# OmerMersin/video-stab

Measured on AMD Instinct MI355X. Metric: stabilized frames/sec @1080p (whole job; warp-stage HBM GB/s in roofline), higher is better.
Workload: dtype u8

## Files before the change

### video-stab_amd/csrc/k_lk.hip

```cpp
#include "vs_common.h"

namespace vsd {
namespace {

constexpr int MAX_LEVELS = 8;

struct LKArgs {
    LKLevel levels[MAX_LEVELS];
    int max_level;
    const float* prev_pts;
    float* next_pts;
    uint8_t* status;
    float* err;
    int n;
    const int32_t* d_n;
    int win;
    int max_count;
    double eps2;
};

template <int CTRL>
__device__ __forceinline__ int dpp_mov(int v) {
    return __builtin_amdgcn_update_dpp(0, v, CTRL, 0xF, 0xF, true);
}
__device__ __forceinline__ int wave_sum_i32(int v) {
    v += dpp_mov<0xB1>(v);
    v += dpp_mov<0x4E>(v);
    v += dpp_mov<0x141>(v);
    v += dpp_mov<0x140>(v);
    return __builtin_amdgcn_readlane(v, 0) + __builtin_amdgcn_readlane(v, 16) +
           __builtin_amdgcn_readlane(v, 32) + __builtin_amdgcn_readlane(v, 48);
}
template <int CTRL>
__device__ __forceinline__ long long dpp_mov64(long long v) {
    const int lo = dpp_mov<CTRL>((int)(unsigned)(unsigned long long)v);
    const int hi = dpp_mov<CTRL>((int)((unsigned long long)v >> 32));
    return (long long)(((unsigned long long)(unsigned)hi << 32) | (unsigned)lo);
}
__device__ __forceinline__ long long wave_sum(int p) {
    long long v = p;
    v += dpp_mov64<0xB1>(v);
    v += dpp_mov64<0x4E>(v);
    v += dpp_mov64<0x141>(v);
    v += dpp_mov64<0x140>(v);
    const int lo = (int)(unsigned)(unsigned long long)v, hi = (int)((unsigned long long)v >> 32);
    long long t = 0;
#pragma unroll
    for (int r = 0; r < 64; r += 16) {
        const unsigned l = (unsigned)__builtin_amdgcn_readlane(lo, r);
        const unsigned h = (unsigned)__builtin_amdgcn_readlane(hi, r);
        t += (long long)(((unsigned long long)h << 32) | l);
    }
    return t;
}

__device__ __forceinline__ int descale(int x, int n) { return (x + (1 << (n - 1))) >> n; }

struct Weights { int w00, w01, w10, w11; };

__device__ __forceinline__ Weights make_weights(float a, float b) {
    Weights w;
    w.w00 = f_round((1.f - a) * (1.f - b) * 16384.f);
    w.w01 = f_round(a * (1.f - b) * 16384.f);
    w.w10 = f_round((1.f - a) * b * 16384.f);
    w.w11 = 16384 - w.w00 - w.w01 - w.w10;
    return w;
}

typedef const __attribute__((address_space(1))) uint8_t* gmem_u8;
__device__ __forceinline__ gmem_u8 uniform_global(const uint8_t* p) {
    const unsigned long long v = (unsigned long long)p;
    const unsigned lo = (unsigned)__builtin_amdgcn_readfirstlane((int)(unsigned)v), hi = (unsigned)__builtin_amdgcn_readfirstlane((int)(unsigned)(v >> 32));
    return (gmem_u8)(((unsigned long long)hi << 32) | lo);
}

constexpr int LK_MARGIN = 6;
constexpr int LK_WIN_MAX = 31;



__device__ __forceinline__ void divmod_small(int i, int d, float inv_d, int& q, int& r) {
    q = (int)(((float)i + 0.5f) * inv_d);
    r = i - q * d;
}

template <int NPX>
__device__ __forceinline__ void lk_track(const LKArgs& a, const int pt) {
    constexpr int WM = NPX <= 4 ? 16 : (NPX <= 7 ? 21 : LK_WIN_MAX);
    constexpr int PWM = WM + 1, RWM = WM + 1 + 2 * LK_MARGIN;
    constexpr int DR = NPX <= 7 ? 3 : 5;
    constexpr int PPM = (PWM + 2 + 3) & ~3;
    constexpr int SRM = (PWM + 1 + 3) / 4, NGM = (PWM + DR - 1) / DR;
    static_assert(SRM * NGM <= 64, "one derivative round per level");
    constexpr int PN = (PPM * (PWM + 2) + 63) / 64, RN = (RWM * RWM + 63) / 64;
    constexpr int PBYTES = (PN * 64 > PPM * (NGM * DR + 2) + 4 ? PN * 64 : PPM * (NGM * DR + 2) + 4);
    __shared__ __attribute__((aligned(16))) uint8_t pI_[4 + PBYTES];
    uint8_t* const pI = pI_ + 4;
    __shared__ __attribute__((aligned(16))) short2 pD[(PWM + 1) * PPM];
    __shared__ uint8_t region[RN * 64];
    const int lane = threadIdx.x;
    int n = a.n;
    if (a.d_n) { int dn = *a.d_n; n = dn < n ? dn : n; }
    if (pt >= n) return;
    const int win = a.win, area = win * win;
    const int PW = win + 1, PP = (PW + 2 + 3) & ~3;
    const int RW = win + 1 + 2 * LK_MARGIN;
    const float inv_pp = 1.0f / (float)PP, inv_rw = 1.0f / (float)RW, inv_win = 1.0f / (float)win;
    uint32_t off[NPX];
#pragma unroll
    for (int k = 0; k < NPX; k++) {
        const int p = lane + 64 * k;
        int yy = 0, xx = 0;
        if (p < area) divmod_small(p, win, inv_win, yy, xx);
        off[k] = (uint32_t)((yy + 1) * PP + xx + 1) | ((uint32_t)(yy * RW + xx) << 16);
    }
#define LK_VALID(k) (lane + 64 * (k) < area)
#define LK_POFF(k) ((int)(off[k] & 0xFFFFu))
#define LK_ROFF(k) ((int)(off[k] >> 16))
    int p_y0, p_x0, p_sy, p_sx, r_y0, r_x0, r_sy, r_sx;
    divmod_small(lane, PP, inv_pp, p_y0, p_x0);
    divmod_small(64, PP, inv_pp, p_sy, p_sx);
    divmod_small(lane, RW, inv_rw, r_y0, r_x0);
    divmod_small(64, RW, inv_rw, r_sy, r_sx);
    const float halfWin = (win - 1) * 0.5f;
    const float FLT_SCALE = 1.f / (1 << 20);
    const float px0 = a.prev_pts[2 * pt], py0 = a.prev_pts[2 * pt + 1];
    float outx = 0.f, outy = 0.f;
    int status = 1;
    float err = 0.f;

    for (int level = a.max_level; level >= 0; level--) {
        const LKLevel L = a.levels[level];
        const float scale = (float)(1. / (double)(1 << level));
        float prevx = px0 * scale, prevy = py0 * scale;
        if (level == a.max_level) { outx = prevx; outy = prevy; }
        else { outx = outx * 2.f; outy = outy * 2.f; }
        prevx -= halfWin; prevy -= halfWin;
        const int ipx = f_floor(prevx), ipy = f_floor(prevy);
        if (ipx < -win || ipx >= L.w || ipy < -win || ipy >= L.h) {
            if (level == 0) { status = 0; err = 0.f; }
            continue;
        }
        float cx = outx - halfWin, cy = outy - halfWin;
        int rx0 = f_floor(cx) - LK_MARGIN, ry0 = f_floor(cy) - LK_MARGIN;
        __syncthreads();
        const int pcount = PP * (PW + 2);
        if (ipx >= 1 && ipy >= 1 && ipx - 1 + PP <= L.w && ipy + PW + 1 <= L.h) {
            const gmem_u8 pbase = uniform_global(L.prev + ((size_t)(ipy - 1) * L.stride + (ipx - 1)));
            constexpr int PB_ = 10;
            int y = p_y0, x = p_x0;
#pragma unroll
            for (int k0 = 0; k0 < PN; k0 += PB_) {
                uint8_t vI[PB_];
#pragma unroll
                for (int k = k0; k < k0 + PB_ && k < PN; k++) {
                    const bool ok = lane + 64 * k < pcount;
                    vI[k - k0] = pbase[ok ? (uint32_t)(y * (int)L.stride + x) : 0u];
                    x += p_sx; y += p_sy;
                    if (x >= PP) { x -= PP; y++; }
                }
#pragma unroll
                for (int k = k0; k < k0 + PB_ && k < PN; k++) pI[lane + 64 * k] = vI[k - k0];
                __builtin_amdgcn_sched_barrier(0);
            }
        } else {
            int y = p_y0, x = p_x0;
            for (int i = lane; i < pcount; i += 64) {
                const int X = ipx - 1 + x, Y = ipy - 1 + y;
                pI[i] = L.prev[(size_t)reflect101(Y, L.h) * L.stride + reflect101(X, L.w)];
                x += p_sx; y += p_sy;
                if (x >= PP) { x -= PP; y++; }
            }
        }
        auto stage_region = [&]() {
            const bool inside = rx0 >= 0 && ry0 >= 0 && rx0 + RW <= L.w && ry0 + RW <= L.h;
            int y = r_y0, x = r_x0;
            asm volatile("" : "+v"(x), "+v"(y));
            if (inside) {
                const gmem_u8 rbase = uniform_global(L.next + ((size_t)ry0 * L.stride + rx0));
                constexpr int RB_ = 10;
#pragma unroll
                for (int k0 = 0; k0 < RN; k0 += RB_) {
                    uint8_t vR[RB_];
#pragma unroll
                    for (int k = k0; k < k0 + RB_ && k < RN; k++) {
                        const bool ok = lane + 64 * k < RW * RW;
                        vR[k - k0] = rbase[ok ? (uint32_t)(y * (int)L.stride + x) : 0u];
                        x += r_sx; y += r_sy;
                        if (x >= RW) { x -= RW; y++; }
                    }
#pragma unroll
                    for (int k = k0; k < k0 + RB_ && k < RN; k++) region[lane + 64 * k] = vR[k - k0];
                    __builtin_amdgcn_sched_barrier(0);
                }
            } else {
                for (int i = lane; i < RW * RW; i += 64) {
                    const int X = rx0 + x, Y = ry0 + y;
                    region[i] = L.next[(size_t)reflect101(Y, L.h) * L.stride + reflect101(X, L.w)];
                    x += r_sx; y += r_sy;
                    if (x >= RW) { x -= RW; y++; }
                }
            }
        };
        stage_region();
        __syncthreads();
        {
            const int sr = (PW + 1 + 3) >> 2;
            int g, c;
            divmod_small(lane, sr, 1.0f / (float)sr, g, c);
            const int y = 1 + g * DR, x = 4 * c;
            if (y <= PW) {
                const bool masked = !(ipx >= 0 && ipy >= 0 && ipx + PW <= L.w && ipy + PW <= L.h);
                int t[3][6];
                auto load_row = [&](int j, int* tj) {
                    const uint32_t* q = reinterpret_cast<const uint32_t*>(pI + j * PP) + c;
                    const uint32_t lo = q[-1], mid = q[0], hi = q[1];
                    tj[0] = lo >> 24;
                    tj[1] = mid & 255u; tj[2] = (mid >> 8) & 255u; tj[3] = (mid >> 16) & 255u; tj[4] = mid >> 24;
                    tj[5] = hi & 255u;
                };
                load_row(y - 1, t[0]);
                load_row(y, t[1]);
#pragma unroll
                for (int r = 0; r < DR; r++) {
                    const int* t0 = t[r % 3];
                    const int* t1 = t[(r + 1) % 3];
                    int* t2 = t[(r + 2) % 3];
                    load_row(y + r + 1, t2);
                    int av[6], bv[6];
#pragma unroll
                    for (int k = 0; k < 6; k++) {
                        av[k] = (t0[k] + t2[k]) * 3 + t1[k] * 10;
                        bv[k] = t2[k] - t0[k];
                    }
                    uint32_t o[4];
#pragma unroll
                    for (int k = 0; k < 4; k++) {
                        const int dx = av[k + 2] - av[k], dy = (bv[k + 2] + bv[k]) * 3 + bv[k + 1] * 10;
                        o[k] = ((uint32_t)dx & 0xFFFFu) | ((uint32_t)dy << 16);
                        if (masked && ((unsigned)(ipx - 1 + x + k) >= (unsigned)L.w || (unsigned)(ipy - 1 + y + r) >= (unsigned)L.h)) o[k] = 0u;
                    }
                    if (y + r <= PW) *reinterpret_cast<uint4*>(&pD[(y + r) * PP + x]) = make_uint4(o[0], o[1], o[2], o[3]);
                    __builtin_amdgcn_sched_barrier(0);
                }
            }
        }
        __syncthreads();
#pragma unroll
        for (int k = 0; k < NPX; k++) asm volatile("" : "+v"(off[k]));
        Weights wt = make_weights(prevx - ipx, prevy - ipy);
        short Iw[NPX], Ix[NPX], Iy[NPX];
        int pA11 = 0, pA12 = 0, pA22 = 0;
#pragma unroll
        for (int k = 0; k < NPX; k++) {
            const int o = LK_POFF(k);
            int ival = descale(__mul24((int)pI[o], wt.w00) + __mul24((int)pI[o + 1], wt.w01) +
                               __mul24((int)pI[o + PP], wt.w10) + __mul24((int)pI[o + PP + 1], wt.w11), 9);
            const short2 d00 = pD[o], d01 = pD[o + 1], d10 = pD[o + PP], d11 = pD[o + PP + 1];
            int ixval = descale(__mul24((int)d00.x, wt.w00) + __mul24((int)d01.x, wt.w01) +
                                __mul24((int)d10.x, wt.w10) + __mul24((int)d11.x, wt.w11), 14);
            int iyval = descale(__mul24((int)d00.y, wt.w00) + __mul24((int)d01.y, wt.w01) +
                                __mul24((int)d10.y, wt.w10) + __mul24((int)d11.y, wt.w11), 14);
            if (!LK_VALID(k)) { ival = 0; ixval = 0; iyval = 0; }
            Iw[k] = (short)ival; Ix[k] = (short)ixval; Iy[k] = (short)iyval;
            pA11 += __mul24(ixval, ixval);
            pA12 += __mul24(ixval, iyval);
            pA22 += __mul24(iyval, iyval);
        }
        const long long sA11 = wave_sum(pA11), sA12 = wave_sum(pA12), sA22 = wave_sum(pA22);
        const float A11 = (float)sA11 * FLT_SCALE, A12 = (float)sA12 * FLT_SCALE, A22 = (float)sA22 * FLT_SCALE;
        float D = A11 * A22 - A12 * A12;
        const float minEig = (A22 + A11 - sqrtf((A11 - A22) * (A11 - A22) + 4.f * A12 * A12)) /
                             (float)(2 * win * win);
        if (minEig < 1e-4f || D < FLT_EPSILON) {
            if (level == 0) status = 0;
            continue;
        }
        D = 1.f / D;
        float pdx = 0.f, pdy = 0.f;
        for (int j = 0; j < a.max_count; j++) {
            const int inx = f_floor(cx), iny = f_floor(cy);
            if (inx < -win || inx >= L.w || iny < -win || iny >= L.h) {
                if (level == 0) status = 0;
                break;
            }
            wt = make_weights(cx - inx, cy - iny);
            int lx = inx - rx0, ly = iny - ry0;
            if (!(lx >= 0 && ly >= 0 && lx + win + 1 <= RW && ly + win + 1 <= RW)) {
                __syncthreads();
                rx0 = inx - LK_MARGIN; ry0 = iny - LK_MARGIN;
                stage_region();
                __syncthreads();
                lx = LK_MARGIN; ly = LK_MARGIN;
            }
            int pb1 = 0, pb2 = 0;
            {
                const int rbase = ly * RW + lx;
#pragma unroll
                for (int k = 0; k < NPX; k++) {
                    const uint8_t* r0 = &region[rbase + LK_ROFF(k)];
                    const int v = descale(__mul24((int)r0[0], wt.w00) + __mul24((int)r0[1], wt.w01) +
                                          __mul24((int)r0[RW], wt.w10) + __mul24((int)r0[RW + 1], wt.w11), 9);
                    const int diff = v - Iw[k];
                    pb1 += __mul24(diff, (int)Ix[k]);
                    pb2 += __mul24(diff, (int)Iy[k]);
                }
            }
            const long long sb1 = wave_sum(pb1), sb2 = wave_sum(pb2);
            const float b1 = (float)sb1 * FLT_SCALE, b2 = (float)sb2 * FLT_SCALE;
            const float dx = (A12 * b2 - A22 * b1) * D;
            const float dy = (A12 * b1 - A11 * b2) * D;
            cx += dx; cy += dy;
            outx = cx + halfWin; outy = cy + halfWin;
            if ((double)dx * (double)dx + (double)dy * (double)dy <= a.eps2) break;
            if (j > 0 && (double)fabsf(dx + pdx) < 0.01 && (double)fabsf(dy + pdy) < 0.01) {
                outx -= dx * 0.5f; outy -= dy * 0.5f;
                break;
            }
            pdx = dx; pdy = dy;
        }
        if (status && level == 0) {
            const float npx = outx - halfWin, npy = outy - halfWin;
            const int inx = f_floor(npx), iny = f_floor(npy);
            if (inx < -win || inx >= L.w || iny < -win || iny >= L.h) {
                status = 0;
            } else {
                wt = make_weights(npx - inx, npy - iny);
                int lx = inx - rx0, ly = iny - ry0;
                if (!(lx >= 0 && ly >= 0 && lx + win + 1 <= RW && ly + win + 1 <= RW)) {
                    __syncthreads();
                    rx0 = inx - LK_MARGIN; ry0 = iny - LK_MARGIN;
                    stage_region();
                    __syncthreads();
                    lx = LK_MARGIN; ly = LK_MARGIN;
                }
                int es = 0;
                {
                    const int rbase = ly * RW + lx;
#pragma unroll
                    for (int k = 0; k < NPX; k++) {
                        const uint8_t* r0 = &region[rbase + LK_ROFF(k)];
                        const int v = descale(__mul24((int)r0[0], wt.w00) + __mul24((int)r0[1], wt.w01) +
                                              __mul24((int)r0[RW], wt.w10) + __mul24((int)r0[RW + 1], wt.w11), 9);
                        const int diff = v - Iw[k];
                        es += LK_VALID(k) ? (diff < 0 ? -diff : diff) : 0;
                    }
                }
                const long long est = wave_sum(es);
                err = (float)est * 1.f / (float)(32 * win * win);
            }
        }
    }
#undef LK_VALID
#undef LK_POFF
#undef LK_ROFF
    if (lane == 0) {
        a.next_pts[2 * pt] = outx;
        a.next_pts[2 * pt + 1] = outy;
        a.status[pt] = (uint8_t)status;
        a.err[pt] = err;
    }
}

template <int NPX>
__global__ __launch_bounds__(64) void lk_kernel(LKArgs a) { lk_track<NPX>(a, blockIdx.x); }

template <int NPX>
__global__ __launch_bounds__(64) void lk_batch_kernel(const LKArgs* __restrict__ table) {
    lk_track<NPX>(table[blockIdx.y], blockIdx.x);
}

int fill_lk_args(LKArgs& a, const LKLevel* levels, int max_level, const float* d_prev_pts, int n, const int32_t* d_n,
                 float* d_next_pts, uint8_t* d_status, float* d_err, int win, int max_iters, double eps) {
    if (!levels || max_level < 0 || max_level >= MAX_LEVELS || n < 0 || win < 3 || win > 31 ||
        !d_prev_pts || !d_next_pts || !d_status || !d_err) {
        set_last_error("pyr_lk: invalid argument (3 <= win <= 31, max_level < 8)");
        return VS_ERR_INVALID_ARG;
    }
    for (int i = 0; i <= max_level; i++) a.levels[i] = levels[i];
    for (int i = max_level + 1; i < MAX_LEVELS; i++) a.levels[i] = levels[max_level];
    a.max_level = max_level;
    a.prev_pts = d_prev_pts; a.next_pts = d_next_pts; a.status = d_status; a.err = d_err;
    a.n = n; a.d_n = d_n; a.win = win;
    a.max_count = max_iters < 0 ? 0 : (max_iters > 100 ? 100 : max_iters);
    double e = eps < 0 ? 0. : (eps > 10. ? 10. : eps);
    a.eps2 = e * e;
    return VS_OK;
}

}

size_t lk_item_bytes() { return sizeof(LKArgs); }

int lk_fill_item(void* host_item, const LKLevel* levels, int max_level, const float* d_prev_pts, int n,
                 const int32_t* d_n, float* d_next_pts, uint8_t* d_status, float* d_err, int win, int max_iters,
                 double eps) {
    return fill_lk_args(*static_cast<LKArgs*>(host_item), levels, max_level, d_prev_pts, n, d_n, d_next_pts, d_status,
                        d_err, win, max_iters, eps);
}

int launch_pyr_lk_batch(const void* d_table, int items, int n_max, int win, hipStream_t st) {
    if (!d_table || items < 1 || items > 65535 || n_max < 0 || win < 3 || win > 31) {
        set_last_error("pyr_lk_batch: invalid argument");
        return VS_ERR_INVALID_ARG;
    }
    if (n_max == 0) return VS_OK;
    const LKArgs* t = static_cast<const LKArgs*>(d_table);
    const int npx = (win * win + 63) / 64;
    dim3 grid(n_max, items), block(64);
    if (npx <= 4) hipLaunchKernelGGL(lk_batch_kernel<4>, grid, block, 0, st, t);
    else if (npx <= 7) hipLaunchKernelGGL(lk_batch_kernel<7>, grid, block, 0, st, t);
    else hipLaunchKernelGGL(lk_batch_kernel<16>, grid, block, 0, st, t);
    VS_HIP_TRY(hipGetLastError());
    return VS_OK;
}

int launch_pyr_lk(const LKLevel* levels, int max_level, const float* d_prev_pts, int n,
                  const int32_t* d_n, float* d_next_pts, uint8_t* d_status, float* d_err, int win,
                  int max_iters, double eps, hipStream_t st) {
    LKArgs a;
    VS_TRY(fill_lk_args(a, levels, max_level, d_prev_pts, n, d_n, d_next_pts, d_status, d_err, win, max_iters, eps));
    if (n == 0) return VS_OK;
    const int npx = (win * win + 63) / 64;
    dim3 grid(n), block(64);
    if (npx <= 4) hipLaunchKernelGGL(lk_kernel<4>, grid, block, 0, st, a);
    else if (npx <= 7) hipLaunchKernelGGL(lk_kernel<7>, grid, block, 0, st, a);
    else hipLaunchKernelGGL(lk_kernel<16>, grid, block, 0, st, a);
    VS_HIP_TRY(hipGetLastError());
    return VS_OK;
}

int run_pyr_lk_op(const uint8_t* d_prev, const uint8_t* d_next, size_t stride, int w, int h,
                  const float* d_prev_pts, int n, float* d_next_pts, uint8_t* d_status,
                  float* d_err, int win, int max_level, int max_iters, double eps, hipStream_t st) {
    if (!d_prev || !d_next || w <= 0 || h <= 0 || max_level < 0 || max_level >= MAX_LEVELS) {
        set_last_error("pyr_lk: invalid argument");
        return VS_ERR_INVALID_ARG;
    }
    int lw[MAX_LEVELS], lh[MAX_LEVELS];
    int levels = 0;
    {
        int sw = w, sh = h;
        for (int level = 0; level <= max_level; level++) {
            lw[level] = sw; lh[level] = sh;
            levels = level;
            sw = (sw + 1) / 2; sh = (sh + 1) / 2;
            if (sw <= win || sh <= win) break;
        }
    }
    size_t img_bytes = 0;
    for (int i = 1; i <= levels; i++) img_bytes += (size_t)lw[i] * lh[i];
    uint8_t* scratch = nullptr;
    VS_HIP_TRY(hipMalloc((void**)&scratch, 2 * img_bytes + 64));
    LKLevel L[MAX_LEVELS];
    uint8_t* pp = scratch;
    uint8_t* pn = scratch + img_bytes;
    int rc = VS_OK;
    for (int i = 0; i <= levels && rc == VS_OK; i++) {
        L[i].w = lw[i]; L[i].h = lh[i];
        if (i == 0) { L[i].prev = d_prev; L[i].next = d_next; L[i].stride = stride; }
        else {
            rc = launch_pyr_down(L[i - 1].prev, L[i - 1].stride, lw[i - 1], lh[i - 1], pp, lw[i], st);
            if (rc == VS_OK) rc = launch_pyr_down(L[i - 1].next, L[i - 1].stride, lw[i - 1], lh[i - 1], pn, lw[i], st);
            L[i].prev = pp; L[i].next = pn; L[i].stride = lw[i];
            pp += (size_t)lw[i] * lh[i]; pn += (size_t)lw[i] * lh[i];
        }
    }
    if (rc == VS_OK) rc = launch_pyr_lk(L, levels, d_prev_pts, n, nullptr, d_next_pts, d_status, d_err, win, max_iters, eps, st);
    hipError_t e = hipStreamSynchronize(st);
    (void)hipFree(scratch);
    if (rc == VS_OK && e != hipSuccess) { set_last_error(hipGetErrorString(e)); rc = VS_ERR_HIP; }
    return rc;
}

}
```

Baseline: 126,300.

## Stage LK patches with 32-bit loads and shorten 64-bit wave reductions

Patch and search-region staging in the pyramidal LK tracker now uses unaligned 32-bit global loads into a row-padded (multiple-of-4) shared layout instead of per-byte loads. This cuts the number of memory instructions per staging pass, and region indexing is updated to the new pitch. The wave reduction now runs its first butterfly steps in 32-bit and only switches to 64-bit when the window size could overflow. This cuts DPP and readlane work per reduction. The padded region reads a few extra columns, which changes the inside-bounds check, and the fallback path now recomputes divmod per element.

```diff
diff --git a/video-stab_amd/csrc/k_lk.hip b/video-stab_amd/csrc/k_lk.hip
--- a/video-stab_amd/csrc/k_lk.hip
+++ b/video-stab_amd/csrc/k_lk.hip
@@ -23,25 +23,33 @@
 __device__ __forceinline__ int dpp_mov(int v) {
     return __builtin_amdgcn_update_dpp(0, v, CTRL, 0xF, 0xF, true);
 }
-__device__ __forceinline__ int wave_sum_i32(int v) {
-    v += dpp_mov<0xB1>(v);
-    v += dpp_mov<0x4E>(v);
-    v += dpp_mov<0x141>(v);
-    v += dpp_mov<0x140>(v);
-    return __builtin_amdgcn_readlane(v, 0) + __builtin_amdgcn_readlane(v, 16) +
-           __builtin_amdgcn_readlane(v, 32) + __builtin_amdgcn_readlane(v, 48);
-}
 template <int CTRL>
 __device__ __forceinline__ long long dpp_mov64(long long v) {
     const int lo = dpp_mov<CTRL>((int)(unsigned)(unsigned long long)v);
     const int hi = dpp_mov<CTRL>((int)((unsigned long long)v >> 32));
     return (long long)(((unsigned long long)(unsigned)hi << 32) | (unsigned)lo);
 }
+constexpr long long LK_LANE_TERM_MAX = 8160ll * 4081ll;
+template <int NPX> struct WaveSumSteps {
+    static constexpr int S = NPX <= 4 ? 4 : (NPX <= 7 ? 3 : 2);
+    static_assert(NPX <= 16 && (long long)NPX * LK_LANE_TERM_MAX * (1 << S) <= 2147483647ll, "the 32-bit butterfly steps must not overflow");
+};
+template <int S>
 __device__ __forceinline__ long long wave_sum(int p) {
-    long long v = p;
-    v += dpp_mov64<0xB1>(v);
-    v += dpp_mov64<0x4E>(v);
-    v += dpp_mov64<0x141>(v);
+    static_assert(S >= 2 && S <= 4, "");
+    unsigned u = (unsigned)p;
+    u += (unsigned)dpp_mov<0xB1>((int)u);
+    u += (unsigned)dpp_mov<0x4E>((int)u);
+    if (S >= 3) u += (unsigned)dpp_mov<0x141>((int)u);
+    if (S >= 4) u += (unsigned)dpp_mov<0x140>((int)u);
+    if (S >= 4) {
+        long long t = 0;
+#pragma unroll
+        for (int r = 0; r < 64; r += 16) t += (long long)__builtin_amdgcn_readlane((int)u, r);
+        return t;
+    }
+    long long v = (int)u;
+    if (S < 3) v += dpp_mov64<0x141>(v);
     v += dpp_mov64<0x140>(v);
     const int lo = (int)(unsigned)(unsigned long long)v, hi = (int)((unsigned long long)v >> 32);
     long long t = 0;
@@ -73,6 +81,9 @@
     const unsigned lo = (unsigned)__builtin_amdgcn_readfirstlane((int)(unsigned)v), hi = (unsigned)__builtin_amdgcn_readfirstlane((int)(unsigned)(v >> 32));
     return (gmem_u8)(((unsigned long long)hi << 32) | lo);
 }
+
+typedef uint32_t __attribute__((aligned(1))) u32_unaligned;
+typedef const __attribute__((address_space(1))) u32_unaligned* gmem_u32u;
 
 constexpr int LK_MARGIN = 6;
 constexpr int LK_WIN_MAX = 31;
@@ -92,12 +103,15 @@
     constexpr int PPM = (PWM + 2 + 3) & ~3;
     constexpr int SRM = (PWM + 1 + 3) / 4, NGM = (PWM + DR - 1) / DR;
     static_assert(SRM * NGM <= 64, "one derivative round per level");
-    constexpr int PN = (PPM * (PWM + 2) + 63) / 64, RN = (RWM * RWM + 63) / 64;
-    constexpr int PBYTES = (PN * 64 > PPM * (NGM * DR + 2) + 4 ? PN * 64 : PPM * (NGM * DR + 2) + 4);
+    constexpr int RDM = (RWM + 3) / 4;
+    constexpr int PN = ((PPM / 4) * (PWM + 2) + 63) / 64, RN = (RDM * RWM + 63) / 64;
+    constexpr int PBYTES = (PN * 256 > PPM * (NGM * DR + 2) + 4 ? PN * 256 : PPM * (NGM * DR + 2) + 4);
+    static_assert((WM - 1) * 4 * RDM + (WM - 1) < 65536 && (WM + 1) * PPM < 65536, "packed window offsets are 16 bits each");
+    constexpr int WS = WaveSumSteps<NPX>::S;
     __shared__ __attribute__((aligned(16))) uint8_t pI_[4 + PBYTES];
     uint8_t* const pI = pI_ + 4;
     __shared__ __attribute__((aligned(16))) short2 pD[(PWM + 1) * PPM];
-    __shared__ uint8_t region[RN * 64];
+    __shared__ __attribute__((aligned(16))) uint8_t region[RN * 256];
     const int lane = threadIdx.x;
     int n = a.n;
     if (a.d_n) { int dn = *a.d_n; n = dn < n ? dn : n; }
@@ -105,6 +119,7 @@
     const int win = a.win, area = win * win;
     const int PW = win + 1, PP = (PW + 2 + 3) & ~3;
     const int RW = win + 1 + 2 * LK_MARGIN;
+    const int PD = PP >> 2, RD = (RW + 3) >> 2, RP = 4 * RD;
     const float inv_pp = 1.0f / (float)PP, inv_rw = 1.0f / (float)RW, inv_win = 1.0f / (float)win;
     uint32_t off[NPX];
 #pragma unroll
@@ -112,16 +127,16 @@
         const int p = lane + 64 * k;
         int yy = 0, xx = 0;
         if (p < area) divmod_small(p, win, inv_win, yy, xx);
-        off[k] = (uint32_t)((yy + 1) * PP + xx + 1) | ((uint32_t)(yy * RW + xx) << 16);
+        off[k] = (uint32_t)((yy + 1) * PP + xx + 1) | ((uint32_t)(yy * RP + xx) << 16);
     }
 #define LK_VALID(k) (lane + 64 * (k) < area)
 #define LK_POFF(k) ((int)(off[k] & 0xFFFFu))
 #define LK_ROFF(k) ((int)(off[k] >> 16))
     int p_y0, p_x0, p_sy, p_sx, r_y0, r_x0, r_sy, r_sx;
-    divmod_small(lane, PP, inv_pp, p_y0, p_x0);
-    divmod_small(64, PP, inv_pp, p_sy, p_sx);
-    divmod_small(lane, RW, inv_rw, r_y0, r_x0);
-    divmod_small(64, RW, inv_rw, r_sy, r_sx);
+    divmod_small(lane, PD, 1.0f / (float)PD, p_y0, p_x0);
+    divmod_small(64, PD, 1.0f / (float)PD, p_sy, p_sx);
+    divmod_small(lane, RD, 1.0f / (float)RD, r_y0, r_x0);
+    divmod_small(64, RD, 1.0f / (float)RD, r_sy, r_sx);
     const float halfWin = (win - 1) * 0.5f;
     const float FLT_SCALE = 1.f / (1 << 20);
     const float px0 = a.prev_pts[2 * pt], py0 = a.prev_pts[2 * pt + 1];
@@ -147,58 +162,48 @@
         const int pcount = PP * (PW + 2);
         if (ipx >= 1 && ipy >= 1 && ipx - 1 + PP <= L.w && ipy + PW + 1 <= L.h) {
             const gmem_u8 pbase = uniform_global(L.prev + ((size_t)(ipy - 1) * L.stride + (ipx - 1)));
-            constexpr int PB_ = 10;
+            uint32_t vI[PN];
             int y = p_y0, x = p_x0;
 #pragma unroll
-            for (int k0 = 0; k0 < PN; k0 += PB_) {
-                uint8_t vI[PB_];
-#pragma unroll
-                for (int k = k0; k < k0 + PB_ && k < PN; k++) {
-                    const bool ok = lane + 64 * k < pcount;
-                    vI[k - k0] = pbase[ok ? (uint32_t)(y * (int)L.stride + x) : 0u];
-                    x += p_sx; y += p_sy;
-                    if (x >= PP) { x -= PP; y++; }
-                }
-#pragma unroll
-                for (int k = k0; k < k0 + PB_ && k < PN; k++) pI[lane + 64 * k] = vI[k - k0];
-                __builtin_amdgcn_sched_barrier(0);
-            }
+            for (int k = 0; k < PN; k++) {
+                const bool ok = lane + 64 * k < (pcount >> 2);
+                vI[k] = *(gmem_u32u)(pbase + (ok ? (uint32_t)(y * (int)L.stride + 4 * x) : 0u));
+                x += p_sx; y += p_sy;
+                if (x >= PD) { x -= PD; y++; }
+            }
+#pragma unroll
+            for (int k = 0; k < PN; k++) reinterpret_cast<uint32_t*>(pI)[lane + 64 * k] = vI[k];
+            __builtin_amdgcn_sched_barrier(0);
         } else {
-            int y = p_y0, x = p_x0;
             for (int i = lane; i < pcount; i += 64) {
+                int y, x;
+                divmod_small(i, PP, inv_pp, y, x);
                 const int X = ipx - 1 + x, Y = ipy - 1 + y;
                 pI[i] = L.prev[(size_t)reflect101(Y, L.h) * L.stride + reflect101(X, L.w)];
-                x += p_sx; y += p_sy;
-                if (x >= PP) { x -= PP; y++; }
             }
         }
         auto stage_region = [&]() {
-            const bool inside = rx0 >= 0 && ry0 >= 0 && rx0 + RW <= L.w && ry0 + RW <= L.h;
+            const bool inside = rx0 >= 0 && ry0 >= 0 && rx0 + RP <= L.w && ry0 + RW <= L.h;
             int y = r_y0, x = r_x0;
             asm volatile("" : "+v"(x), "+v"(y));
             if (inside) {
                 const gmem_u8 rbase = uniform_global(L.next + ((size_t)ry0 * L.stride + rx0));
-                constexpr int RB_ = 10;
-#pragma unroll
-                for (int k0 = 0; k0 < RN; k0 += RB_) {
-                    uint8_t vR[RB_];
-#pragma unroll
-                    for (int k = k0; k < k0 + RB_ && k < RN; k++) {
-                        const bool ok = lane + 64 * k < RW * RW;
-                        vR[k - k0] = rbase[ok ? (uint32_t)(y * (int)L.stride + x) : 0u];
-                        x += r_sx; y += r_sy;
-                        if (x >= RW) { x -= RW; y++; }
-                    }
-#pragma unroll
-                    for (int k = k0; k < k0 + RB_ && k < RN; k++) region[lane + 64 * k] = vR[k - k0];
-                    __builtin_amdgcn_sched_barrier(0);
-                }
+                uint32_t vR[RN];
+#pragma unroll
+                for (int k = 0; k < RN; k++) {
+                    const bool ok = lane + 64 * k < RD * RW;
+                    vR[k] = *(gmem_u32u)(rbase + (ok ? (uint32_t)(y * (int)L.stride + 4 * x) : 0u));
+                    x += r_sx; y += r_sy;
+                    if (x >= RD) { x -= RD; y++; }
+                }
+#pragma unroll
+                for (int k = 0; k < RN; k++) reinterpret_cast<uint32_t*>(region)[lane + 64 * k] = vR[k];
+                __builtin_amdgcn_sched_barrier(0);
             } else {
                 for (int i = lane; i < RW * RW; i += 64) {
+                    divmod_small(i, RW, inv_rw, y, x);
                     const int X = rx0 + x, Y = ry0 + y;
-                    region[i] = L.next[(size_t)reflect101(Y, L.h) * L.stride + reflect101(X, L.w)];
-                    x += r_sx; y += r_sy;
-                    if (x >= RW) { x -= RW; y++; }
+                    region[y * RP + x] = L.next[(size_t)reflect101(Y, L.h) * L.stride + reflect101(X, L.w)];
                 }
             }
         };
@@ -267,7 +272,7 @@
             pA12 += __mul24(ixval, iyval);
             pA22 += __mul24(iyval, iyval);
         }
-        const long long sA11 = wave_sum(pA11), sA12 = wave_sum(pA12), sA22 = wave_sum(pA22);
+        const long long sA11 = wave_sum<WS>(pA11), sA12 = wave_sum<WS>(pA12), sA22 = wave_sum<WS>(pA22);
         const float A11 = (float)sA11 * FLT_SCALE, A12 = (float)sA12 * FLT_SCALE, A22 = (float)sA22 * FLT_SCALE;
         float D = A11 * A22 - A12 * A12;
         const float minEig = (A22 + A11 - sqrtf((A11 - A22) * (A11 - A22) + 4.f * A12 * A12)) /
@@ -295,18 +300,18 @@
             }
             int pb1 = 0, pb2 = 0;
             {
-                const int rbase = ly * RW + lx;
+                const int rbase = ly * RP + lx;
 #pragma unroll
                 for (int k = 0; k < NPX; k++) {
                     const uint8_t* r0 = &region[rbase + LK_ROFF(k)];
                     const int v = descale(__mul24((int)r0[0], wt.w00) + __mul24((int)r0[1], wt.w01) +
-                                          __mul24((int)r0[RW], wt.w10) + __mul24((int)r0[RW + 1], wt.w11), 9);
+                                          __mul24((int)r0[RP], wt.w10) + __mul24((int)r0[RP + 1], wt.w11), 9);
                     const int diff = v - Iw[k];
                     pb1 += __mul24(diff, (int)Ix[k]);
                     pb2 += __mul24(diff, (int)Iy[k]);
                 }
             }
-            const long long sb1 = wave_sum(pb1), sb2 = wave_sum(pb2);
+            const long long sb1 = wave_sum<WS>(pb1), sb2 = wave_sum<WS>(pb2);
             const float b1 = (float)sb1 * FLT_SCALE, b2 = (float)sb2 * FLT_SCALE;
             const float dx = (A12 * b2 - A22 * b1) * D;
             const float dy = (A12 * b1 - A11 * b2) * D;
@@ -336,17 +341,17 @@
                 }
                 int es = 0;
                 {
-                    const int rbase = ly * RW + lx;
+                    const int rbase = ly * RP + lx;
 #pragma unroll
                     for (int k = 0; k < NPX; k++) {
                         const uint8_t* r0 = &region[rbase + LK_ROFF(k)];
                         const int v = descale(__mul24((int)r0[0], wt.w00) + __mul24((int)r0[1], wt.w01) +
-                                              __mul24((int)r0[RW], wt.w10) + __mul24((int)r0[RW + 1], wt.w11), 9);
+                                              __mul24((int)r0[RP], wt.w10) + __mul24((int)r0[RP + 1], wt.w11), 9);
                         const int diff = v - Iw[k];
                         es += LK_VALID(k) ? (diff < 0 ? -diff : diff) : 0;
                     }
                 }
-                const long long est = wave_sum(es);
+                const long long est = wave_sum<WS>(es);
                 err = (float)est * 1.f / (float)(32 * win * win);
             }
         }
```

Measured after the change: 130,500, median of 6. 3.3% higher.
